# GabrieleCocco/CLFaceDetection

Hardware: NVIDIA B200
Metric: frames_per_sec_1080p (higher is better)
Workload: dtype f64

## Files before the change

clfacedetection_b200/csrc/haar_pack.cpp:

```cpp
#include <algorithm>
#include <cfloat>
#include <cmath>
#include <cstdarg>
#include <cstdio>
#include <cstdlib>
#include <cstring>

#include "clfd_pack.h"

namespace clfd {

static thread_local char g_error[1024] = "";

void set_error(const char *fmt, ...) {
    va_list ap;
    va_start(ap, fmt);
    vsnprintf(g_error, sizeof g_error, fmt, ap);
    va_end(ap);
}
const char *get_error() { return g_error; }

#define FMT_FAIL(...) do { set_error(__VA_ARGS__); return CLFD_ERR_FORMAT; } while (0)

int build_hidden(HostCascade &c) {
// ... 165 lines not shown
    L.eq_off[2] = (ey + eh) * pitch + ex; L.eq_off[3] = (ey + eh) * pitch + ex + ew;
    for (int n = 0; n < c.n_nodes(); n++) {
        const HostNode &nd = c.nodes[n];
        ScNode &d = out[n];
        memset(&d, 0, sizeof d);
        const int nr = c.hid_nrects[n];
        double sum0 = 0, area0 = 0;
        const double correction_ratio = weight_scale * (!nd.tilted ? 1 : 0.5);
        for (int k = 0; k < nr; k++) {
            const int tx = cv_round_d(nd.rect[k][0] * scale), tw = cv_round_d(nd.rect[k][2] * scale);
            const int ty = cv_round_d(nd.rect[k][1] * scale), th = cv_round_d(nd.rect[k][3] * scale);
            int dy[4], dx[4];
            if (!nd.tilted) {
                dy[0] = ty;      dx[0] = tx;
                dy[1] = ty;      dx[1] = tx + tw;
                dy[2] = ty + th; dx[2] = tx;
                dy[3] = ty + th; dx[3] = tx + tw;
            } else {
                dy[2] = ty + tw;      dx[2] = tx + tw;
                dy[3] = ty + tw + th; dx[3] = tx + tw - th;
                dy[0] = ty;           dx[0] = tx;
                dy[1] = ty + th;      dx[1] = tx - th;
            }
            for (int q = 0; q < 4; q++) d.off[k * 4 + q] = dy[q] * pitch + dx[q];
            d.w[k] = (float)(nd.weight[k] * correction_ratio);
            if (k == 0) area0 = tw * th;
            else sum0 += d.w[k] * tw * th;
        }
        d.w[0] = (float)(-sum0 / area0);
        d.thr = nd.threshold;
        d.left = nd.left; d.right = nd.right;
        d.flags = (nd.tilted ? 1 : 0) | (nr << 8);
    }
}

static void pack_dense_one(const HostCascade &c, int ystep, DenseParams &P, std::vector<TailStump> &tail,
                           std::vector<DenseStage> &stage_tab, int &dense_stumps, int patch_stride = 0,
                           bool allow_tiles = true) {
    const int S = c.n_stages(), T = c.n_trees();
    memset(&P, 0, sizeof P);
    P.total_stages = S;
    P.win_w = c.win_w; P.win_h = c.win_h;
    P.tile_stride = dense_tile_stride(c.win_w, ystep);
    P.tile_half = dense_tile_half(c.win_w, ystep);
    if (patch_stride > 0) { P.tile_stride = patch_stride; P.tile_half = 0; }
    P.is_tree = c.is_tree ? 1 : 0;
    P.ystep = ystep;
    P.filter_eps = 9.5367431640625e-07f;
    if (const char *e = getenv("CLFD_FORCE_EXACT")) P.force_exact = atoi(e) != 0;
    P.inv_area = 1. / ((c.win_w - 2) * (c.win_h - 2));
    P.eq_x = 1; P.eq_y = 1; P.eq_w = c.win_w - 2; P.eq_h = c.win_h - 2;
    P.tilted_tile = c.has_tilted && !getenv("CLFD_NO_TILTED_TILE") ? 1 : 0;
    P.tile_h = kTileH;
    if (P.tilted_tile && ystep == 2 && !c.is_tree && !getenv("CLFD_NO_SMALL_TILES")) P.tile_h = kTileHSmall;
    if (ystep == 2 && !P.tilted_tile && !c.is_tree && c.is_stump_based) {
        const char *e = getenv("CLFD_TILE_H2");
        if (!e || atoi(e) == 24) P.tile_h = 24;
    }
    const size_t tile_bytes = (size_t)dense_tile_rows(c.win_h, ystep, P.tile_h) * P.tile_stride * 4;
    const size_t tilt_base = (tile_bytes + 127) & ~(size_t)127;
    const bool dense_ok = allow_tiles && tile_bytes <= 65536 && (!P.tilted_tile || 2 * tilt_base <= 160 * 1024) && c.win_w <= 255 && c.win_h <= 255;
    int npt = 1;
    for (int t = 0; t < T; t++) npt = std::max(npt, c.tr_nnodes[t]);
    if (getenv("CLFD_NO_NODE_TILES") && npt > 1) npt = kMaxTreeNodes + 1;
    P.npt = npt <= kMaxTreeNodes ? npt : 1;
    auto stage_ok = [&](int i) {
// ... 75 lines not shown
                for (int k = 0; k < c.hid_nrects[n]; k++) {
                    int dx[4], dy[4];
                    corner_coords(nd, k, dx, dy);
                    for (int q = 0; q < 4; q++) ts.off[k * 4 + q] = tile_offset(dy[q], dx[q]) + (nd.tilted ? (uint32_t)tilt_base : 0u);
                    ts.w[k] = c.hid_weight[(size_t)n * 3 + k];
                }
                ts.thr = nd.threshold;
                ts.a0 = nd.left <= 0 ? c.alpha[a + (-nd.left)] : 0.f;
                ts.a1 = nd.right <= 0 ? c.alpha[a + (-nd.right)] : 0.f;
                ts.meta = (uint32_t)j | ((nd.left > 0 ? (uint32_t)nd.left : kNodeLeaf) << 8) |
                          ((nd.right > 0 ? (uint32_t)nd.right : kNodeLeaf) << 16);
                amax = fmax(amax, fmax(fabs((double)ts.a0), fabs((double)ts.a1)));
            }
            abs_sum += amax;
        }
        ds.first = 0; ds.count = (uint16_t)(c.st_ntrees[i] * P.npt);
        ds.thr = c.hid_thr[i];
        ds.flags = ((!c.is_tree && c.is_stump_based && c.two_rects[i]) ? 1u : 0u) | (any3 ? 2u : 0u) |
                   (c.order_free[i] ? 4u : 0u);
        const double er = (double)(c.st_ntrees[i] * P.npt) * ldexp(1.0, -23) * abs_sum;
        ds.sum_eps = std::isfinite(er) ? (float)(er * 1.0000002) + FLT_MIN : INFINITY;
        ds.sum_eps += 1.0001e-5f * std::fabs(ds.thr);
        if (walk_tree) {
            const uint32_t pass = c.st_child[i] >= 0 ? (uint32_t)pos[c.st_child[i]] : kRouteAccept;
            int p = i;
            while (p >= 0 && c.st_next[p] < 0) p = c.st_parent[p];
            const uint32_t fail = p >= 0 ? (uint32_t)pos[c.st_next[p]] : kRouteReject;
            ds.flags |= ((uint32_t)i << 8) | (pass << 16) | (fail << 24);
            stage_tab[e] = ds;
        }
        if (e < elig) P.stage[e] = ds;
    }
    const bool share_corners = !getenv("CLFD_NO_SHARED_CORNERS");
    int ns = 0, nstump = 0;
    while (ns < elig && nstump + c.st_ntrees[ns] * P.npt <= kMaxDenseStumps) {
        P.stage[ns].first = (uint16_t)nstump;
        std::vector<DenseStump> six, rest;
        for (int t = c.st_first_tree[ns] * P.npt; t < c.st_first_tree[ns + 1] * P.npt; t++) {
            DenseStump st = tail[t];
            bool shared = false;
            if (share_corners && P.npt == 1 && c.hid_nrects[c.tr_first_node[t]] == 2) {
                const uint32_t *A = st.off, *B = st.off + 4;
                static const int pairs[4][2] = {{0, 2}, {3, 1}, {0, 1}, {3, 2}};
                for (const auto &pr : pairs) {
                    const int pl = pr[0], mi = pr[1];
                    if (A[pl] != B[pl] || A[mi] != B[mi]) continue;
                    const int opl = pl == 0 ? 3 : 0, omi = mi == 1 ? 2 : 1;
                    const uint32_t o[6] = {A[pl], A[mi], A[opl], A[omi], B[opl], B[omi]};
                    for (int q = 0; q < 12; q++) st.off[q] = q < 6 ? o[q] : 0;
                    shared = true;
                    break;
                }
            }
            (shared ? six : rest).push_back(st);
        }
        P.stage[ns].n_shared = (uint32_t)six.size();
        for (const auto &st : six) P.stump[nstump++] = st;
        for (const auto &st : rest) P.stump[nstump++] = st;
        ns++;
    }
    P.n_stages = ns;
    {
        static_assert(sizeof(TailStump) == 80, "five 16-byte chunks per record");
        struct Chunk { uint32_t v[4]; };
        std::vector<TailStump> blocked;
        const Chunk *src = reinterpret_cast<const Chunk *>(tail.data());
        int at = 0;
        for (int e = 0; e < E; e++) {
            const int count = c.st_ntrees[order[e]] * P.npt;
            const size_t first = blocked.size();
            blocked.resize(first + (size_t)((count + 31) / 32) * 32);
            Chunk *blk = reinterpret_cast<Chunk *>(blocked.data() + first);
            for (int j = 0; j < count; j++)
                for (int q = 0; q < 5; q++) blk[(size_t)(j >> 5) * 160 + q * 32 + (j & 31)] = src[(size_t)(at + j) * 5 + q];
            if (e < elig) P.stage[e].tail_first = (uint32_t)first;
            if (walk_tree) stage_tab[e].tail_first = (uint32_t)first;
            at += count;
        }
        tail.swap(blocked);
    }
    P.pool_min = 0;
    if (const char *e = getenv("CLFD_POOL_MIN")) P.pool_min = std::max(0, atoi(e));
    P.track_abs = 0;
    for (float v : c.alpha)
        if (std::fabs(v) > 64.f) P.track_abs = 1;
    if (getenv("CLFD_NO_TRACK_ABS")) P.track_abs = 0;
// ... 100 lines not shown
```

clfacedetection_b200/csrc/kernels_clod.cu:

```cuda
#include <algorithm>
#include <cstdint>

#include "clfd_pack.h"
#include "kernels.h"

namespace clfd {

typedef unsigned long long ull;

__device__ __forceinline__ uint32_t smem_u32(const void *p) { return (uint32_t)__cvta_generic_to_shared(p); }

__device__ __forceinline__ void mbar_init(uint64_t *bar, uint32_t count) {
    asm volatile("mbarrier.init.shared::cta.b64 [%0], %1;" ::"r"(smem_u32(bar)), "r"(count));
    asm volatile("fence.mbarrier_init.release.cluster;" ::: "memory");
}
__device__ __forceinline__ void mbar_expect_tx(uint64_t *bar, uint32_t bytes) {
    asm volatile("mbarrier.arrive.expect_tx.shared::cta.b64 _, [%0], %1;" ::"r"(smem_u32(bar)), "r"(bytes) : "memory");
}
__device__ __forceinline__ void mbar_wait(uint64_t *bar, uint32_t parity) {
    asm volatile(
        "{\n"
        ".reg .pred P1;\n"
        "LAB_WAIT:\n"
        "mbarrier.try_wait.parity.shared::cta.b64 P1, [%0], %1;\n"
// ... 177 lines not shown
    const double sigma = dense_sigma(P, c, wid);
    const uint4 *rec = reinterpret_cast<const uint4 *>(P.tail + tail_first);
    double S = 0.0;
    uint32_t at = 0;
    for (int j = 0; j < count; j++) {
        const StumpRegs q = stump_from_global(rec, j, true);
        if (NODES) {
            if ((q.meta & 255u) == 0u) at = 0;
            if ((q.meta & 255u) != at) continue;
        }
        const int r0 = lds32(base + q.o[0]) - lds32(base + q.o[1]) - lds32(base + q.o[2]) + lds32(base + q.o[3]);
        const int r1 = lds32(base + q.o[4]) - lds32(base + q.o[5]) - lds32(base + q.o[6]) + lds32(base + q.o[7]);
        const double t = __dmul_rn((double)q.thr, sigma);
        double sum;
        if (dbl) {
            sum = __fma_rn((double)r1, (double)q.w1, __dmul_rn((double)r0, (double)q.w0));
        } else {
            sum = __dadd_rn((double)__fmul_rn(__int2float_rn(r0), q.w0), (double)__fmul_rn(__int2float_rn(r1), q.w1));
            if (q.o[11] != 0) {
                const int r2 = lds32(base + q.o[8]) - lds32(base + q.o[9]) - lds32(base + q.o[10]) + lds32(base + q.o[11]);
                sum = __dadd_rn(sum, (double)__fmul_rn(__int2float_rn(r2), q.w2));
            }
        }
        if (NODES) {
            at = ((sum >= t ? q.meta >> 16 : q.meta >> 8)) & 255u;
            if (at != kNodeLeaf) continue;
        }
        S = __dadd_rn(S, (double)(sum >= t ? q.a1 : q.a0));
    }
    const double thr = (double)sthr;
    return (S >= thr ? 1 : 0) | (fabs(__dsub_rn(S, thr)) <= __dmul_rn(1e-5, fabs(thr)) ? 2 : 0);
}

template <int KK, int K, bool FIXED, int ROWSTEP, bool SHARED, bool NODES, bool TRACK>
__device__ __forceinline__ void stump_filter_window(const StumpRegs &q, bool dbl, bool three, float eps, const uint32_t (&c)[12],
                                                    const uint32_t (&base)[K], const float (&sg)[K], float (&S)[K], bool (&near)[K],
                                                    uint32_t (&at)[K], float (&Sa)[K]) {
    const float eps4 = eps * 0.25f;
    constexpr int IMM = KK * ROWSTEP;
    const uint32_t b = base[FIXED ? 0 : KK];
    int r0, r1;
    if (SHARED) {
        int e, f, g;
        if (FIXED) {
            e = lds32i<IMM>(c[0]) - lds32i<IMM>(c[1]); f = lds32i<IMM>(c[2]) - lds32i<IMM>(c[3]); g = lds32i<IMM>(c[4]) - lds32i<IMM>(c[5]);
        } else {
            e = lds32(b + q.o[0]) - lds32(b + q.o[1]); f = lds32(b + q.o[2]) - lds32(b + q.o[3]); g = lds32(b + q.o[4]) - lds32(b + q.o[5]);
        }
        r0 = e + f; r1 = e + g;
    } else if (FIXED) {
        r0 = lds32i<IMM>(c[0]) - lds32i<IMM>(c[1]) - lds32i<IMM>(c[2]) + lds32i<IMM>(c[3]);
        r1 = lds32i<IMM>(c[4]) - lds32i<IMM>(c[5]) - lds32i<IMM>(c[6]) + lds32i<IMM>(c[7]);
    } else {
        r0 = lds32(b + q.o[0]) - lds32(b + q.o[1]) - lds32(b + q.o[2]) + lds32(b + q.o[3]);
        r1 = lds32(b + q.o[4]) - lds32(b + q.o[5]) - lds32(b + q.o[6]) + lds32(b + q.o[7]);
    }
    const float p0 = __fmul_rn(__int2float_rn(r0), q.w0);
    float s32 = __fmaf_rn(__int2float_rn(r1), q.w1, p0);
    float m = __fmaf_rn(fabsf(p0), eps4, __fmul_rn(fabsf(q.thr), __fmul_rn(sg[KK], eps)));
    if (!SHARED && three) {
        int r2;
        if (FIXED) r2 = lds32i<IMM>(c[8]) - lds32i<IMM>(c[9]) - lds32i<IMM>(c[10]) + lds32i<IMM>(c[11]);
        else r2 = lds32(b + q.o[8]) - lds32(b + q.o[9]) - lds32(b + q.o[10]) + lds32(b + q.o[11]);
        m = __fmaf_rn(fabsf(s32), eps4, m);
        s32 = __fmaf_rn(__int2float_rn(r2), q.w2, s32);
    }
    const float d = __fmaf_rn(-q.thr, sg[KK], s32);
    if (NODES) {
        const bool on = at[KK] == (q.meta & 255u);
        near[KK] = near[KK] || (on && fabsf(d) <= m);
        S[KK] = __fadd_rn(S[KK], on ? (d >= 0.f ? q.a1 : q.a0) : 0.f);
        at[KK] = on ? ((d >= 0.f ? q.meta >> 16 : q.meta >> 8) & 255u) : at[KK];
    } else {
        near[KK] = near[KK] || (fabsf(d) <= m);
        const float sel = d >= 0.f ? q.a1 : q.a0;
        S[KK] = __fadd_rn(S[KK], sel);
        if (TRACK) Sa[KK] = __fadd_rn(Sa[KK], fabsf(sel));
    }
}

template <int K, bool FIXED, int ROWSTEP, bool SHARED, bool NODES, bool TRACK>
__device__ __forceinline__ void stump_filter(const StumpRegs &q, bool dbl, bool any3, float eps, const uint32_t (&base)[K],
                                             const float (&sg)[K], float (&S)[K], bool (&near)[K], uint32_t (&at)[K], float (&Sa)[K]) {
    static_assert(K >= 1 && K <= 4, "1..4 windows per thread");
    const bool three = !SHARED && any3 && q.o[11] != 0u;
    uint32_t c[12];
    if (FIXED) {
#pragma unroll
        for (int i = 0; i < (SHARED ? 6 : 12); i++) c[i] = base[0] + q.o[i];
    }
    if (NODES && (q.meta & 255u) == 0u) {
#pragma unroll
        for (int k = 0; k < K; k++) at[k] = 0u;
    }
    stump_filter_window<0, K, FIXED, ROWSTEP, SHARED, NODES, TRACK>(q, dbl, three, eps, c, base, sg, S, near, at, Sa);
    if (K > 1) stump_filter_window<(K > 1 ? 1 : 0), K, FIXED, ROWSTEP, SHARED, NODES, TRACK>(q, dbl, three, eps, c, base, sg, S, near, at, Sa);
    if (K > 2) stump_filter_window<(K > 2 ? 2 : 0), K, FIXED, ROWSTEP, SHARED, NODES, TRACK>(q, dbl, three, eps, c, base, sg, S, near, at, Sa);
    if (K > 3) stump_filter_window<(K > 3 ? 3 : 0), K, FIXED, ROWSTEP, SHARED, NODES, TRACK>(q, dbl, three, eps, c, base, sg, S, near, at, Sa);
}

template <int K, bool FIXED, int ROWSTEP, bool NODES, bool TRACK>
__device__ __forceinline__ void stage_filter(const DenseParams &P, const DenseStage &st, bool resident, int grp, int G,
                                             const uint32_t (&base)[K], const float (&sg)[K], float (&S)[K], bool (&near)[K],
                                             float (&Sa)[K]) {
    uint32_t at[K];
#pragma unroll
    for (int k = 0; k < K; k++) at[k] = 0u;
    const int count = st.count;
    const uint32_t flags = st.flags;
    const bool dbl = flags & 1u, any3 = flags & 2u;
    const float eps = P.filter_eps;
    if (resident && G == 1) {
        const int first = st.first, n6 = (int)st.n_shared;
#pragma unroll 1
        for (int j = 0; j < n6; j++) stump_filter<K, FIXED, ROWSTEP, true, false, TRACK>(stump_from_param(P.stump[first + j]), dbl, false, eps, base, sg, S, near, at, Sa);
#pragma unroll 1
        for (int j = n6; j < count; j++) stump_filter<K, FIXED, ROWSTEP, false, NODES, TRACK>(stump_from_param(P.stump[first + j]), dbl, any3, eps, base, sg, S, near, at, Sa);
    } else {
        const uint4 *__restrict__ rec = reinterpret_cast<const uint4 *>(P.tail + st.tail_first);
        if (NODES) {
            const int npt = P.npt;
#pragma unroll 1
            for (int j = grp * npt; j < count; j += G * npt)
#pragma unroll 1
                for (int i = 0; i < npt; i++)
                    stump_filter<K, FIXED, ROWSTEP, false, true, TRACK>(stump_from_global(rec, j + i, any3), dbl, any3, eps, base, sg, S, near, at, Sa);
        } else {
#pragma unroll 1
            for (int j = grp; j < count; j += G) stump_filter<K, FIXED, ROWSTEP, false, false, TRACK>(stump_from_global(rec, j, any3), dbl, any3, eps, base, sg, S, near, at, Sa);
        }
    }
// ... 80 lines not shown
            if (tid == 0) mbar_init(bar, 1);
            __syncthreads();
            const uint32_t hb = (uint32_t)half * 4u;
            if (tid == 0) mbar_expect_tx(bar, (uint32_t)rows * 2u * hb);
            const int32_t *__restrict__ gdi = a.sum + frame_off + (size_t)py0 * L.sum_pitch + (px0 >> 1);
            for (int r = tid; r < rows * 2; r += kDenseThreads) {
                const int odd = r >= rows, rr = odd ? r - rows : r;
                tma_bulk_g2s(tile + (size_t)rr * S * 4 + (odd ? hb : 0u), gdi + (size_t)rr * L.sum_pitch + (odd ? (L.sum_pitch >> 1) : 0), hb, bar);
            }
        }
        const int c4 = cols >> 2, total = rows * c4;
        for (int i = (di ? total : 0) + tid; i < total * n_tiles_smem; i += kDenseThreads) {
            const int t2 = i >= total, ii = t2 ? i - total : i;
            const int r = ii / c4, cq = ii - r * c4;
            const int4 v = __ldg(reinterpret_cast<const int4 *>((t2 ? gtil : gsum) + (size_t)r * L.sum_pitch) + cq);
            int *row = reinterpret_cast<int *>(tile + (t2 ? tile2_off : 0)) + r * S;
            *reinterpret_cast<int2 *>(row + 2 * cq) = make_int2(v.x, v.z);
            *reinterpret_cast<int2 *>(row + half + 2 * cq) = make_int2(v.y, v.w);
        }
        __syncthreads();
        if (di) mbar_wait(bar, 0);
    }

    DenseCtx c;
    c.tile = smem_u32(tile); c.gsq = a.sq; c.sq_at = frame_off + (size_t)py0 * L.sum_pitch + px0; c.sq32 = a.sq32 != 0;
    c.codes = a.codes ? a.codes + (size_t)frame * a.windows_per_frame + CL.win_base : nullptr;
    c.sq_pitch = L.sum_pitch;
    c.row_mul = ystep * S * 4;
    c.ystep = ystep; c.S = S; c.half = P.tile_half;
    c.tx = tx; c.wy_tile = ty * TILE_H; c.nx = CL.nx;
    c.code_mul = P.is_tree ? 2 : 1;
    const float inf = __int_as_float(0x7f800000);

    constexpr int kRowsPerSlot = kDenseThreads / kTileW;
    const int wx = tid & (kTileW - 1), wy0 = tid / kTileW;
    uint32_t alive = 0;
#pragma unroll
    for (int k = 0; k < kDenseSlots; k++) {
        const int wy = wy0 + k * kRowsPerSlot;
        const int wid = wy * kTileW + wx;
        if (wx < n_wx && wy < n_wy) {
            bool eq_flat, live = true;
            sgf[wid] = (float)dense_sigma_flat(P, c, wid, eq_flat);
            if (!COUNT && eq_flat && P.flat_code) {
                const int code = flat_window_code(P, c, wid);
                if (code != kNotFlat) {
                    live = false;
                    if (P.is_tree ? (code & 1) : (code == P.total_stages)) emit_rect(a, CL, frame, px0 + wx * ystep, py0 + wy * ystep);
                }
            }
            if (live) alive |= 1u << k;
        } else {
            sgf[wid] = 1.0f;
        }
    }
    int s = 0;
    for (; s < P.n_fixed; s++) {
        const float sthr = P.stage[s].thr, seps = P.force_exact ? inf : P.stage[s].sum_eps;
#pragma unroll 1
        for (int k0 = 0; k0 < kDenseSlots; k0 += kDenseChunk) {
            const uint32_t m4 = (alive >> k0) & ((1u << kDenseChunk) - 1u);
            if (!__any_sync(0xffffffffu, m4 != 0)) continue;
            uint32_t base[kDenseChunk];
            float sg[kDenseChunk];
            float Ssum[kDenseChunk];
            bool near[kDenseChunk];
#pragma unroll
            for (int k = 0; k < kDenseChunk; k++) {
                const int wy = wy0 + (k0 + k) * kRowsPerSlot;
                base[k] = c.tile + (uint32_t)(wy * c.row_mul + wx * 4);
                sg[k] = sgf[wy * kTileW + wx];
                Ssum[k] = 0.f;
                near[k] = false;
            }
            float Sabs[kDenseChunk];
#pragma unroll
            for (int k = 0; k < kDenseChunk; k++) Sabs[k] = 0.f;
            if (ROWSTEP_T) stage_filter<kDenseChunk, true, ROWSTEP_T, NODES, TRACK>(P, P.stage[s], true, 0, 1, base, sg, Ssum, near, Sabs);
            else stage_filter<kDenseChunk, false, 0, NODES, TRACK>(P, P.stage[s], true, 0, 1, base, sg, Ssum, near, Sabs);
#pragma unroll
            for (int k = 0; k < kDenseChunk; k++) {
                if (!((m4 >> k) & 1u)) continue;
                const int wid = (wy0 + (k0 + k) * kRowsPerSlot) * kTileW + wx;
                if (!stage_verdict<NODES, COUNT, TRACK>(P, c, P.stage[s], sthr, seps, wid, Ssum[k], near[k], Sabs[k])) {
                    alive &= ~(1u << (k0 + k));
                    if (c.codes) dense_write_code(c, wid, s * c.code_mul);
                }
            }
        }
    }

    constexpr int kClassCap = kTileWindows / 32;
    constexpr int kSeg = kTileWindows / kDenseWarps;
    int n_alive;
    uint16_t *cur;
    if (kPooledStages && P.pool_min > 0) {
        uint16_t *cl_in = list, *cl_out = reinterpret_cast<uint16_t *>(smem_raw + plan.pool);
        int *cnt_in = ctl + kCtlCount, *cnt_out = ctl + kCtlCountB, *cnt_zero = ctl + kCtlCountC;
        {
            const int na = __popc(alive);
            if (na) {
                const int cq = (wx + 8 * wy0) & 31;
                int at = atomicAdd(cnt_in + cq, na);
    #pragma unroll
                for (int k = 0; k < kDenseSlots; k++)
                    if ((alive >> k) & 1u) cl_in[cq * kClassCap + at++] = (uint16_t)((wy0 + k * kRowsPerSlot) * kTileW + wx);
            }
        }
        __syncthreads();
            for (;; s++) {
            const int h = cnt_in[lane];
            int incl = h, hmax = h;
    #pragma unroll
            for (int d = 1; d < 32; d <<= 1) {
                const int v = __shfl_up_sync(0xffffffffu, incl, d);
                if (lane >= d) incl += v;
                hmax = max(hmax, __shfl_xor_sync(0xffffffffu, hmax, d));
            }
            const int excl = incl - h, tot = __shfl_sync(0xffffffffu, incl, 31);
            if (tot == 0) return;
            n_alive = tot;
            if (!(P.pool_min > 0 && tot > P.pool_min && s < P.tail_stages)) {
                for (int r = warp; r < h; r += kDenseWarps) {
                    const int i = excl + r;
                    const int w = i % kDenseWarps, p = i / kDenseWarps;
                    const int nw = (tot - w + kDenseWarps - 1) / kDenseWarps, Rw = (nw + 31) >> 5;
                    const int col = p / Rw, row = p - col * Rw;
                    cl_out[w * kSeg + row * 32 + col] = cl_in[lane * kClassCap + r];
                }
                __syncthreads();
                break;
            }
            int R = (tot + 31) >> 5;
            {
                int best = 0x7fffffff;
                for (int r = R; r <= hmax; r++) {
                    int e = max(h - r, 0);
    #pragma unroll
                    for (int d = 16; d > 0; d >>= 1) e += __shfl_xor_sync(0xffffffffu, e, d);
// ... 25 lines not shown
                }
                if (valid && !pass && c.codes) dense_write_code(c, wid, s * c.code_mul);
            };
            for (int r = r_begin; r < r_end; r += 2) {
                bool v0, v1 = false;
                const int wid0 = fetch(r, v0);
                if (r + 1 < r_end) {
                    const int wid1 = fetch(r + 1, v1);
                    const uint32_t base[2] = {dense_base(c, wid0), dense_base(c, wid1)};
                    const float sg[2] = {sgf[wid0], sgf[wid1]};
                    float Ssum[2] = {0.f, 0.f};
                    bool near[2] = {false, false};
                    float Sabs[2] = {0.f, 0.f};
                    stage_filter<2, false, 0, NODES, TRACK>(P, P.stage[s], s < P.n_stages, 0, 1, base, sg, Ssum, near, Sabs);
                    keep_pool(v0, wid0, Ssum[0], near[0], Sabs[0]);
                    keep_pool(v1, wid1, Ssum[1], near[1], Sabs[1]);
                } else {
                    const uint32_t base[1] = {dense_base(c, wid0)};
                    const float sg[1] = {sgf[wid0]};
                    float Ssum[1] = {0.f};
                    bool near[1] = {false};
                    float Sabs[1] = {0.f};
                    stage_filter<1, false, 0, NODES, TRACK>(P, P.stage[s], s < P.n_stages, 0, 1, base, sg, Ssum, near, Sabs);
                    keep_pool(v0, wid0, Ssum[0], near[0], Sabs[0]);
                }
            }
            __syncthreads();
            uint16_t *tl = cl_in; cl_in = cl_out; cl_out = tl;
            int *tc = cnt_in; cnt_in = cnt_out; cnt_out = cnt_zero; cnt_zero = tc;
        }

        cur = cl_out + warp * kSeg;
    } else {
        const int na = __popc(alive), cq = (wx + 8 * wy0) & 31;
        int at = na ? atomicAdd(ctl + kCtlCount + cq, na) : 0;
        __syncthreads();
        const int h = ctl[kCtlCount + lane];
        int incl = h;
#pragma unroll
        for (int d = 1; d < 32; d <<= 1) {
            const int v = __shfl_up_sync(0xffffffffu, incl, d);
            if (lane >= d) incl += v;
        }
        n_alive = __shfl_sync(0xffffffffu, incl, 31);
        if (n_alive == 0) return;
        at += __shfl_sync(0xffffffffu, incl - h, cq);
#pragma unroll
        for (int k = 0; k < kDenseSlots; k++) {
            if ((alive >> k) & 1u) {
                const int i = at++;
                const int w = i % kDenseWarps, p = i / kDenseWarps;
                const int nw = (n_alive - w + kDenseWarps - 1) / kDenseWarps, Rw = (nw + 31) >> 5;
                const int col = p / Rw, row = p - col * Rw;
                list[w * kSeg + row * 32 + col] = (uint16_t)((wy0 + k * kRowsPerSlot) * kTileW + wx);
            }
        }
        __syncthreads();
        cur = list + warp * kSeg;
    }

#ifdef CLFD_TILE_TIMING
    if (lane == 0) atomicAdd(&s_dense_t_p1, (unsigned int)(clock64() - t_start));
#endif
    int n = (n_alive - warp + kDenseWarps - 1) / kDenseWarps;
    bool dealt = true;
    for (; s < P.cut_stages && n > 0; s++) {
        const float sthr = P.stage[s].thr, seps = P.force_exact ? inf : P.stage[s].sum_eps;
        int n_next = 0;
        auto keep = [&](bool valid, int wid, float Ssum, bool near, float Sabs) {
            const bool pass = valid && stage_verdict<NODES, COUNT, TRACK>(P, c, P.stage[s], sthr, seps, wid, Ssum, near, Sabs);
            const unsigned m = __ballot_sync(0xffffffffu, pass);
            if (pass) cur[n_next + __popc(m & ((1u << lane) - 1u))] = (uint16_t)wid;
            n_next += __popc(m);
            if (valid && !pass && c.codes) dense_write_code(c, wid, s * c.code_mul);
        };
        if (n > P.g1_min) {
            const int R = (n + 31) >> 5;
            for (int r = 0; r < R; r += 2) {
                const int c0 = dealt ? (n - r + R - 1) / R : min(32, n - 32 * r);
                if (r + 1 < R) {
                    const int c1 = dealt ? (n - r - 1 + R - 1) / R : min(32, n - 32 * (r + 1));
                    const bool v0 = lane < c0, v1 = lane < c1;
                    const int wid0 = cur[32 * r + (v0 ? lane : 0)], wid1 = cur[32 * r + 32 + (v1 ? lane : 0)];
                    __syncwarp();
                    const uint32_t base[2] = {dense_base(c, wid0), dense_base(c, wid1)};
                    const float sg[2] = {sgf[wid0], sgf[wid1]};
                    float Ssum[2] = {0.f, 0.f};
// ... 135 lines not shown
            }
            __syncwarp();
        }
        return;
    }
    if (n == 0) return;
    ull qb = 0;
    if (s < P.total_stages) {
        if (lane == 0) qb = atomicAdd(a.qcount, (ull)n);
        qb = __shfl_sync(0xffffffffu, qb, 0);
    }
    const int Rn = (n + 31) >> 5;
    for (int idx = lane; idx < Rn * 32; idx += 32) {
        const int row = idx >> 5, col = idx & 31;
        if (col >= (dealt ? (n - row + Rn - 1) / Rn : min(32, n - 32 * row))) continue;
        const int i = dealt ? col * Rn + row : idx;
        const int w = cur[idx];
        const int x = px0 + (w & (kTileW - 1)) * ystep, y = py0 + (w / kTileW) * ystep;
        if (s >= P.total_stages) {
            emit_rect(a, CL, frame, x, y);
            if (c.codes) dense_write_code(c, w, P.total_stages);
        } else if (qb + i < a.queue_cap) {
            QueueItem it;
            it.key = ((uint32_t)frame << 16) | ((uint32_t)cl << 8) | (uint32_t)s;
            it.xy = ((uint32_t)y << 16) | (uint32_t)x;
            a.queue[qb + i] = it;
        } else {
            atomicAdd(a.counters + 3, 1ull);
        }
    }
}

template <int ROWSTEP_T, bool TREE, bool NODES, int TILE_H, bool COUNT, bool TRACK = false>
__global__ void __launch_bounds__(kDenseThreads)
k_cascade_tiles(const __grid_constant__ DenseParams P, const __grid_constant__ CascadeArgs a, const int tile0) {
    extern __shared__ __align__(128) unsigned char smem_raw[];
#ifdef CLFD_TILE_TIMING
    const long long t_cta = clock64();
#endif
    cascade_tiles_body<ROWSTEP_T, TREE, NODES, TILE_H, COUNT, TRACK>(P, a, tile0, smem_raw);
#ifdef CLFD_TILE_TIMING
    __syncwarp();
    if ((threadIdx.x & 31) == 0) {
        const unsigned int dt = (unsigned int)(clock64() - t_cta);
        atomicAdd(&s_dense_t_busy, dt);
        __threadfence_block();
        if (atomicAdd(&s_dense_done, 1u) == kDenseWarps - 1) {
            atomicAdd(a.counters + 4, (ull)s_dense_t_busy);
            atomicAdd(a.counters + 5, (ull)dt * kDenseWarps);
            atomicAdd(a.counters + 6, (ull)s_dense_t_p1);
        }
    }
    return;
#endif
    if (!COUNT) return;
    __syncwarp();
    if ((threadIdx.x & 31) == 0) {
        __threadfence_block();
        if (atomicAdd(&s_dense_done, 1u) == kDenseWarps - 1) {
            const unsigned int ne = s_dense_exact, nn = s_dense_near;
            if (ne) atomicAdd(a.counters + 4, (ull)ne);
            if (nn) atomicAdd(a.counters + 5, (ull)nn);
        }
    }
}

constexpr int kPatchWarps = 8;
// ... 111 lines not shown
            if (alive) emit_rect(a, CL, frame, x, y);
            if (c.codes) dense_write_code(c, 0, alive ? P.total_stages : s);
        }
        __syncwarp();
        q = qn;
    }
    if (!COUNT) return;
    __syncwarp();
    if (lane == 0) {
        __threadfence_block();
        if (atomicAdd(&s_dense_done, 1u) == kPatchWarps - 1) {
            const unsigned int ne = s_dense_exact, nn = s_dense_near;
            if (ne) atomicAdd(a.counters + 4, (ull)ne);
            if (nn) atomicAdd(a.counters + 5, (ull)nn);
        }
    }
}
static cudaError_t launch_patch_tt(const DenseParams &P, const CascadeArgs &a, int n_sms, cudaStream_t stream) {
    const size_t smem = (size_t)kPatchWarps * 2 * patch_buf_words(P) * 4;
    static SmemLimitCache limit;
    if (cudaError_t e = limit.ensure(k_cascade_patch<kTilesCount>, smem)) return e;
    const int per_sm = (int)std::max<size_t>(1, std::min<size_t>(4, (200 * 1024) / std::max<size_t>(smem, 1)));
    k_cascade_patch<kTilesCount><<<n_sms * per_sm, 32 * kPatchWarps, smem, stream>>>(P, a);
    return cudaGetLastError();
}

constexpr int dense_stride_ce(int win_w, int ystep) {
    int cols = ((kTileW - 1) * ystep + win_w + 1 + 3) & ~3;
    int s = ystep == 1 ? cols : 2 * ((cols / 2 + 3) & ~3);
    s = (s + 3) & ~3;
    while ((ystep * s) % 32 != 8) s += 4;
    return s;
}
constexpr int dense_rowstep_ce(int win_w, int ystep) { return (kDenseThreads / kTileW) * ystep * dense_stride_ce(win_w, ystep) * 4; }

template <int ROWSTEP_T, bool TREE, bool NODES, int TILE_H = kTileH>
static cudaError_t launch_tiles_tt(const DenseParams &P, const CascadeArgs &a, int tile0, int n_tiles, size_t smem, cudaStream_t stream) {
    if constexpr (ROWSTEP_T == 0 && !TREE && !NODES) {
        if (P.track_abs) {
            static SmemLimitCache limit_track;
            if (cudaError_t e = limit_track.ensure(k_cascade_tiles<0, false, false, TILE_H, kTilesCount, true>, smem)) return e;
            k_cascade_tiles<0, false, false, TILE_H, kTilesCount, true><<<dim3(n_tiles, a.n_frames), kDenseThreads, smem, stream>>>(P, a, tile0);
            return cudaGetLastError();
        }
    }
    static SmemLimitCache limit;
    if (cudaError_t e = limit.ensure(k_cascade_tiles<ROWSTEP_T, TREE, NODES, TILE_H, kTilesCount>, smem)) return e;
    k_cascade_tiles<ROWSTEP_T, TREE, NODES, TILE_H, kTilesCount><<<dim3(n_tiles, a.n_frames), kDenseThreads, smem, stream>>>(P, a, tile0);
    return cudaGetLastError();
}
template <int ROWSTEP_T>
static cudaError_t launch_tiles_t(const DenseParams &P, const CascadeArgs &a, int tile0, int n_tiles, size_t smem, cudaStream_t stream) {
    constexpr int R = ROWSTEP_T;
    if (P.exec_stages > P.tail_stages) return launch_tiles_tt<R, true, false>(P, a, tile0, n_tiles, smem, stream);
    if (P.tile_h == kTileHSmall) {
        if (P.npt > 1) return launch_tiles_tt<R, false, true, kTileHSmall>(P, a, tile0, n_tiles, smem, stream);
        return launch_tiles_tt<R, false, false, kTileHSmall>(P, a, tile0, n_tiles, smem, stream);
    }
    if (P.tile_h == 24) {
        if (P.exec_stages > P.tail_stages || P.npt > 1) return cudaErrorInvalidValue;
        return launch_tiles_tt<ROWSTEP_T, false, false, 24>(P, a, tile0, n_tiles, smem, stream);
    }
    if (P.tile_h != kTileH) return cudaErrorInvalidValue;
    if (P.npt > 1) return launch_tiles_tt<R, false, true>(P, a, tile0, n_tiles, smem, stream);
    return launch_tiles_tt<ROWSTEP_T, false, false>(P, a, tile0, n_tiles, smem, stream);
}

#ifdef CLFD_TILES_COUNT_TU
cudaError_t launch_cascade_patch_count(const DenseParams &P, const CascadeArgs &a, int n_sms, cudaStream_t stream) {
    return launch_patch_tt(P, a, n_sms, stream);
}
#else
cudaError_t launch_cascade_patch_count(const DenseParams &P, const CascadeArgs &a, int n_sms, cudaStream_t stream);
cudaError_t launch_cascade_patch(const DenseParams &P, const CascadeArgs &a, int n_sms, cudaStream_t stream) {
    if (a.n_frames == 0) return cudaSuccess;
    return a.count_exact ? launch_cascade_patch_count(P, a, n_sms, stream) : launch_patch_tt(P, a, n_sms, stream);
}
#endif
#ifdef CLFD_TILES_COUNT_TU
cudaError_t launch_cascade_tiles_count(const DenseParams &P, const CascadeArgs &a, int tile0, int n_tiles, cudaStream_t stream) {
#else
cudaError_t launch_cascade_tiles_count(const DenseParams &P, const CascadeArgs &a, int tile0, int n_tiles, cudaStream_t stream);
cudaError_t launch_cascade_tiles(const DenseParams &P, const CascadeArgs &a, int tile0, int n_tiles, cudaStream_t stream) {
    if (a.count_exact) return launch_cascade_tiles_count(P, a, tile0, n_tiles, stream);
#endif
    if (n_tiles <= 0 || a.n_frames == 0) return cudaSuccess;
    const size_t smem = dense_smem_plan(P).total;
    const int rowstep = (kDenseThreads / kTileW) * P.ystep * P.tile_stride * 4;
    constexpr int r20_1 = dense_rowstep_ce(20, 1), r20_2 = dense_rowstep_ce(20, 2);
    constexpr int r24_1 = dense_rowstep_ce(24, 1), r24_2 = dense_rowstep_ce(24, 2);
    static_assert(r20_1 == r24_1 && r20_2 == r24_2 && r20_2 != r20_1, "row steps must be distinct switch labels");
    if (P.track_abs && P.exec_stages <= P.tail_stages && P.npt == 1) return launch_tiles_t<0>(P, a, tile0, n_tiles, smem, stream);
    switch (rowstep) {
        case r20_1: return launch_tiles_t<r20_1>(P, a, tile0, n_tiles, smem, stream);
        case r20_2: return launch_tiles_t<r20_2>(P, a, tile0, n_tiles, smem, stream);
        default:    return launch_tiles_t<0>(P, a, tile0, n_tiles, smem, stream);
    }
}

#ifndef CLFD_TILES_COUNT_TU
__global__ void __launch_bounds__(256) k_enqueue_all(const CascadeArgs a) {
    const long long w = (long long)blockIdx.x * 256 + threadIdx.x;
    const int frame = blockIdx.y;
    if (w == 0 && frame == 0) a.counters[1] = (ull)a.windows_per_frame * a.n_frames;
    if (w >= a.windows_per_frame) return;
    int lo = 0, hi = a.n_cas_levels - 1;
    while (lo < hi) {
        const int mid = (lo + hi + 1) >> 1;
        if (__ldg(&a.cas_levels[mid].win_base) <= w) lo = mid; else hi = mid - 1;
    }
    const int nx = __ldg(&a.cas_levels[lo].nx), ystep = __ldg(&a.cas_levels[lo].ystep);
    const int local = (int)(w - __ldg(&a.cas_levels[lo].win_base));
    const int iy = local / nx, ix = local - iy * nx;
    QueueItem it;
    it.key = ((uint32_t)frame << 16) | ((uint32_t)lo << 8);
    it.xy = ((uint32_t)(iy * ystep) << 16) | (uint32_t)(ix * ystep);
    a.queue[(size_t)frame * a.windows_per_frame + w] = it;
}

cudaError_t launch_enqueue_all(const CascadeArgs &a, cudaStream_t stream) {
    if (a.windows_per_frame == 0 || a.n_frames == 0) return cudaSuccess;
// ... 279 lines not shown
```

Measured before the change: 2852.

## Assign consecutive window rows per thread and reuse rectangle pair sums across rows

Each thread now handles vertically adjacent windows instead of rows strided by the thread-row count, so per-slot row offset becomes a single ystep row. The host packer computes a per-stump descriptor recording when one rectangle corner-pair difference equals another pair shifted down by 1-3 rows. In the fixed-offset kernel path, already loaded pair differences from earlier slots are reused instead of reloaded from shared memory. This cuts shared-memory loads but adds registers (h[6][K]); launch bounds now request min-blocks occupancy. The compaction class assignment is also reworked for the new mapping.

After: 2558, median of 6. -10.3%, worse.

```diff
diff --git a/clfacedetection_b200/csrc/haar_pack.cpp b/clfacedetection_b200/csrc/haar_pack.cpp
--- a/clfacedetection_b200/csrc/haar_pack.cpp
+++ b/clfacedetection_b200/csrc/haar_pack.cpp
@@ -221,6 +221,20 @@
         d.left = nd.left; d.right = nd.right;
         d.flags = (nd.tilted ? 1 : 0) | (nr << 8);
     }
+}
+
+static uint32_t reuse_descriptor(const uint32_t off[12], bool six, int64_t row_bytes) {
+    auto shift = [&](int p, int s) -> uint32_t {
+        const int64_t d0 = (int64_t)off[2 * s] - off[2 * p], d1 = (int64_t)off[2 * s + 1] - off[2 * p + 1];
+        if (d0 != d1 || d0 <= 0 || d0 % row_bytes != 0 || d0 / row_bytes > 3) return 0u;
+        return (uint32_t)(d0 / row_bytes);
+    };
+    if (six) {
+        uint32_t mef = shift(0, 1), meg = shift(0, 2);
+        if (mef && meg) (mef <= meg ? meg : mef) = 0u;
+        return mef | (meg << 2) | (shift(1, 0) << 4) | (shift(2, 0) << 6);
+    }
+    return shift(0, 1) | (shift(2, 3) << 2) | (off[11] != 0u ? shift(4, 5) << 4 : 0u);
 }
 
 static void pack_dense_one(const HostCascade &c, int ystep, DenseParams &P, std::vector<TailStump> &tail,
@@ -362,6 +376,7 @@
         if (e < elig) P.stage[e] = ds;
     }
     const bool share_corners = !getenv("CLFD_NO_SHARED_CORNERS");
+    const int64_t row_bytes = (int64_t)ystep * P.tile_stride * 4;
     int ns = 0, nstump = 0;
     while (ns < elig && nstump + c.st_ntrees[ns] * P.npt <= kMaxDenseStumps) {
         P.stage[ns].first = (uint16_t)nstump;
@@ -376,12 +391,13 @@
                     const int pl = pr[0], mi = pr[1];
                     if (A[pl] != B[pl] || A[mi] != B[mi]) continue;
                     const int opl = pl == 0 ? 3 : 0, omi = mi == 1 ? 2 : 1;
-                    const uint32_t o[6] = {A[pl], A[mi], A[opl], A[omi], B[opl], B[omi]};
+                    const uint32_t o[6] = {A[pl], A[mi], A[omi], A[opl], B[omi], B[opl]};
                     for (int q = 0; q < 12; q++) st.off[q] = q < 6 ? o[q] : 0;
                     shared = true;
                     break;
                 }
             }
+            if (P.npt == 1) st.meta = reuse_descriptor(st.off, shared, row_bytes);
             (shared ? six : rest).push_back(st);
         }
         P.stage[ns].n_shared = (uint32_t)six.size();
diff --git a/clfacedetection_b200/csrc/kernels_clod.cu b/clfacedetection_b200/csrc/kernels_clod.cu
--- a/clfacedetection_b200/csrc/kernels_clod.cu
+++ b/clfacedetection_b200/csrc/kernels_clod.cu
@@ -233,22 +233,60 @@
     return (S >= thr ? 1 : 0) | (fabs(__dsub_rn(S, thr)) <= __dmul_rn(1e-5, fabs(thr)) ? 2 : 0);
 }
 
+constexpr uint32_t kMaxPairShift = 2u;
+template <int KK>
+__device__ __forceinline__ bool pair_reusable(uint32_t m) { return KK > 0 && m != 0u && m <= (uint32_t)KK && m <= kMaxPairShift; }
+template <int KK, int K>
+__device__ __forceinline__ int pair_from(const int (&h)[K], uint32_t m) {
+    int v = h[KK >= 1 ? KK - 1 : 0];
+    if (KK >= 2 && m == 2u) v = h[KK >= 2 ? KK - 2 : 0];
+    if (KK >= 3 && kMaxPairShift >= 3 && m == 3u) v = h[KK >= 3 ? KK - 3 : 0];
+    return v;
+}
+template <int KK, int K, int ROWSTEP, int PP>
+__device__ __forceinline__ int pair_load(const uint32_t (&c)[12], int (&h)[6][K]) {
+    const int v = lds32i<KK * ROWSTEP>(c[2 * PP]) - lds32i<KK * ROWSTEP>(c[2 * PP + 1]);
+    h[PP][KK] = v;
+    return v;
+}
+template <int KK, int K, int ROWSTEP, int PP, int SRC>
+__device__ __forceinline__ int pair_reuse(const uint32_t (&c)[12], int (&h)[6][K], uint32_t m) {
+    if (pair_reusable<KK>(m)) {
+        const int v = pair_from<KK, K>(h[SRC], m);
+        h[PP][KK] = v;
+        return v;
+    }
+    return pair_load<KK, K, ROWSTEP, PP>(c, h);
+}
+
 template <int KK, int K, bool FIXED, int ROWSTEP, bool SHARED, bool NODES, bool TRACK>
 __device__ __forceinline__ void stump_filter_window(const StumpRegs &q, bool dbl, bool three, float eps, const uint32_t (&c)[12],
                                                     const uint32_t (&base)[K], const float (&sg)[K], float (&S)[K], bool (&near)[K],
-                                                    uint32_t (&at)[K], float (&Sa)[K]) {
+                                                    uint32_t (&at)[K], float (&Sa)[K], int (&h)[6][K]) {
     const float eps4 = eps * 0.25f;
     constexpr int IMM = KK * ROWSTEP;
+    constexpr bool REUSE = FIXED && !NODES;
     const uint32_t b = base[FIXED ? 0 : KK];
     int r0, r1;
     if (SHARED) {
         int e, f, g;
-        if (FIXED) {
+        if (REUSE) {
+            const uint32_t d = q.meta, mef = d & 3u, meg = (d >> 2) & 3u;
+            if (pair_reusable<KK>(mef)) { e = pair_from<KK, K>(h[1], mef); h[0][KK] = e; }
+            else if (pair_reusable<KK>(meg)) { e = pair_from<KK, K>(h[2], meg); h[0][KK] = e; }
+            else e = pair_load<KK, K, ROWSTEP, 0>(c, h);
+            f = pair_reuse<KK, K, ROWSTEP, 1, 0>(c, h, (d >> 4) & 3u);
+            g = pair_reuse<KK, K, ROWSTEP, 2, 0>(c, h, (d >> 6) & 3u);
+        } else if (FIXED) {
             e = lds32i<IMM>(c[0]) - lds32i<IMM>(c[1]); f = lds32i<IMM>(c[2]) - lds32i<IMM>(c[3]); g = lds32i<IMM>(c[4]) - lds32i<IMM>(c[5]);
         } else {
             e = lds32(b + q.o[0]) - lds32(b + q.o[1]); f = lds32(b + q.o[2]) - lds32(b + q.o[3]); g = lds32(b + q.o[4]) - lds32(b + q.o[5]);
         }
-        r0 = e + f; r1 = e + g;
+        r0 = e - f; r1 = e - g;
+    } else if (REUSE) {
+        const uint32_t d = q.meta;
+        r0 = pair_reuse<KK, K, ROWSTEP, 0, 1>(c, h, d & 3u) - pair_load<KK, K, ROWSTEP, 1>(c, h);
+        r1 = pair_reuse<KK, K, ROWSTEP, 2, 3>(c, h, (d >> 2) & 3u) - pair_load<KK, K, ROWSTEP, 3>(c, h);
     } else if (FIXED) {
         r0 = lds32i<IMM>(c[0]) - lds32i<IMM>(c[1]) - lds32i<IMM>(c[2]) + lds32i<IMM>(c[3]);
         r1 = lds32i<IMM>(c[4]) - lds32i<IMM>(c[5]) - lds32i<IMM>(c[6]) + lds32i<IMM>(c[7]);
@@ -261,7 +299,8 @@
     float m = __fmaf_rn(fabsf(p0), eps4, __fmul_rn(fabsf(q.thr), __fmul_rn(sg[KK], eps)));
     if (!SHARED && three) {
         int r2;
-        if (FIXED) r2 = lds32i<IMM>(c[8]) - lds32i<IMM>(c[9]) - lds32i<IMM>(c[10]) + lds32i<IMM>(c[11]);
+        if (REUSE) r2 = pair_reuse<KK, K, ROWSTEP, 4, 5>(c, h, (q.meta >> 4) & 3u) - pair_load<KK, K, ROWSTEP, 5>(c, h);
+        else if (FIXED) r2 = lds32i<IMM>(c[8]) - lds32i<IMM>(c[9]) - lds32i<IMM>(c[10]) + lds32i<IMM>(c[11]);
         else r2 = lds32(b + q.o[8]) - lds32(b + q.o[9]) - lds32(b + q.o[10]) + lds32(b + q.o[11]);
         m = __fmaf_rn(fabsf(s32), eps4, m);
         s32 = __fmaf_rn(__int2float_rn(r2), q.w2, s32);
@@ -294,10 +333,11 @@
 #pragma unroll
         for (int k = 0; k < K; k++) at[k] = 0u;
     }
-    stump_filter_window<0, K, FIXED, ROWSTEP, SHARED, NODES, TRACK>(q, dbl, three, eps, c, base, sg, S, near, at, Sa);
-    if (K > 1) stump_filter_window<(K > 1 ? 1 : 0), K, FIXED, ROWSTEP, SHARED, NODES, TRACK>(q, dbl, three, eps, c, base, sg, S, near, at, Sa);
-    if (K > 2) stump_filter_window<(K > 2 ? 2 : 0), K, FIXED, ROWSTEP, SHARED, NODES, TRACK>(q, dbl, three, eps, c, base, sg, S, near, at, Sa);
-    if (K > 3) stump_filter_window<(K > 3 ? 3 : 0), K, FIXED, ROWSTEP, SHARED, NODES, TRACK>(q, dbl, three, eps, c, base, sg, S, near, at, Sa);
+    int h[6][K];
+    stump_filter_window<0, K, FIXED, ROWSTEP, SHARED, NODES, TRACK>(q, dbl, three, eps, c, base, sg, S, near, at, Sa, h);
+    if (K > 1) stump_filter_window<(K > 1 ? 1 : 0), K, FIXED, ROWSTEP, SHARED, NODES, TRACK>(q, dbl, three, eps, c, base, sg, S, near, at, Sa, h);
+    if (K > 2) stump_filter_window<(K > 2 ? 2 : 0), K, FIXED, ROWSTEP, SHARED, NODES, TRACK>(q, dbl, three, eps, c, base, sg, S, near, at, Sa, h);
+    if (K > 3) stump_filter_window<(K > 3 ? 3 : 0), K, FIXED, ROWSTEP, SHARED, NODES, TRACK>(q, dbl, three, eps, c, base, sg, S, near, at, Sa, h);
 }
 
 template <int K, bool FIXED, int ROWSTEP, bool NODES, bool TRACK>
@@ -444,12 +484,11 @@
     c.code_mul = P.is_tree ? 2 : 1;
     const float inf = __int_as_float(0x7f800000);
 
-    constexpr int kRowsPerSlot = kDenseThreads / kTileW;
-    const int wx = tid & (kTileW - 1), wy0 = tid / kTileW;
+    const int wx = tid & (kTileW - 1), wy1 = (tid / kTileW) * kDenseSlots;
     uint32_t alive = 0;
 #pragma unroll
     for (int k = 0; k < kDenseSlots; k++) {
-        const int wy = wy0 + k * kRowsPerSlot;
+        const int wy = wy1 + k;
         const int wid = wy * kTileW + wx;
         if (wx < n_wx && wy < n_wy) {
             bool eq_flat, live = true;
@@ -479,7 +518,7 @@
             bool near[kDenseChunk];
 #pragma unroll
             for (int k = 0; k < kDenseChunk; k++) {
-                const int wy = wy0 + (k0 + k) * kRowsPerSlot;
+                const int wy = wy1 + k0 + k;
                 base[k] = c.tile + (uint32_t)(wy * c.row_mul + wx * 4);
                 sg[k] = sgf[wy * kTileW + wx];
                 Ssum[k] = 0.f;
@@ -493,7 +532,7 @@
 #pragma unroll
             for (int k = 0; k < kDenseChunk; k++) {
                 if (!((m4 >> k) & 1u)) continue;
-                const int wid = (wy0 + (k0 + k) * kRowsPerSlot) * kTileW + wx;
+                const int wid = (wy1 + k0 + k) * kTileW + wx;
                 if (!stage_verdict<NODES, COUNT, TRACK>(P, c, P.stage[s], sthr, seps, wid, Ssum[k], near[k], Sabs[k])) {
                     alive &= ~(1u << (k0 + k));
                     if (c.codes) dense_write_code(c, wid, s * c.code_mul);
@@ -504,19 +543,23 @@
 
     constexpr int kClassCap = kTileWindows / 32;
     constexpr int kSeg = kTileWindows / kDenseWarps;
+    constexpr int kClassesPerThread = kDenseSlots < 4 ? kDenseSlots : 4;
+    constexpr uint32_t kClassSlots = 0x11u;
     int n_alive;
     uint16_t *cur;
     if (kPooledStages && P.pool_min > 0) {
         uint16_t *cl_in = list, *cl_out = reinterpret_cast<uint16_t *>(smem_raw + plan.pool);
         int *cnt_in = ctl + kCtlCount, *cnt_out = ctl + kCtlCountB, *cnt_zero = ctl + kCtlCountC;
         {
-            const int na = __popc(alive);
-            if (na) {
-                const int cq = (wx + 8 * wy0) & 31;
-                int at = atomicAdd(cnt_in + cq, na);
     #pragma unroll
-                for (int k = 0; k < kDenseSlots; k++)
-                    if ((alive >> k) & 1u) cl_in[cq * kClassCap + at++] = (uint16_t)((wy0 + k * kRowsPerSlot) * kTileW + wx);
+            for (int j = 0; j < kClassesPerThread; j++) {
+                const uint32_t mine = alive & (kClassSlots << j);
+                if (!mine) continue;
+                const int cq = (wx + 8 * (wy1 + j)) & 31;
+                int at = atomicAdd(cnt_in + cq, __popc(mine));
+    #pragma unroll
+                for (int k = j; k < kDenseSlots; k += 4)
+                    if ((mine >> k) & 1u) cl_in[cq * kClassCap + at++] = (uint16_t)((wy1 + k) * kTileW + wx);
             }
         }
         __syncthreads();
@@ -608,8 +651,12 @@
 
         cur = cl_out + warp * kSeg;
     } else {
-        const int na = __popc(alive), cq = (wx + 8 * wy0) & 31;
-        int at = na ? atomicAdd(ctl + kCtlCount + cq, na) : 0;
+        int at[kClassesPerThread];
+#pragma unroll
+        for (int j = 0; j < kClassesPerThread; j++) {
+            const int na = __popc(alive & (kClassSlots << j));
+            at[j] = na ? atomicAdd(ctl + kCtlCount + ((wx + 8 * (wy1 + j)) & 31), na) : 0;
+        }
         __syncthreads();
         const int h = ctl[kCtlCount + lane];
         int incl = h;
@@ -620,15 +667,17 @@
         }
         n_alive = __shfl_sync(0xffffffffu, incl, 31);
         if (n_alive == 0) return;
-        at += __shfl_sync(0xffffffffu, incl - h, cq);
+#pragma unroll
+        for (int j = 0; j < kClassesPerThread; j++)
+            at[j] += __shfl_sync(0xffffffffu, incl - h, (wx + 8 * (wy1 + j)) & 31);
 #pragma unroll
         for (int k = 0; k < kDenseSlots; k++) {
             if ((alive >> k) & 1u) {
-                const int i = at++;
+                const int i = at[k & 3]++;
                 const int w = i % kDenseWarps, p = i / kDenseWarps;
                 const int nw = (n_alive - w + kDenseWarps - 1) / kDenseWarps, Rw = (nw + 31) >> 5;
                 const int col = p / Rw, row = p - col * Rw;
-                list[w * kSeg + row * 32 + col] = (uint16_t)((wy0 + k * kRowsPerSlot) * kTileW + wx);
+                list[w * kSeg + row * 32 + col] = (uint16_t)((wy1 + k) * kTileW + wx);
             }
         }
         __syncthreads();
@@ -830,7 +879,7 @@
 }
 
 template <int ROWSTEP_T, bool TREE, bool NODES, int TILE_H, bool COUNT, bool TRACK = false>
-__global__ void __launch_bounds__(kDenseThreads)
+__global__ void __launch_bounds__(kDenseThreads, TREE || (TRACK && TILE_H != 24) ? 3 : NODES ? 0 : 4)
 k_cascade_tiles(const __grid_constant__ DenseParams P, const __grid_constant__ CascadeArgs a, const int tile0) {
     extern __shared__ __align__(128) unsigned char smem_raw[];
 #ifdef CLFD_TILE_TIMING
@@ -1008,7 +1057,7 @@
     while ((ystep * s) % 32 != 8) s += 4;
     return s;
 }
-constexpr int dense_rowstep_ce(int win_w, int ystep) { return (kDenseThreads / kTileW) * ystep * dense_stride_ce(win_w, ystep) * 4; }
+constexpr int dense_rowstep_ce(int win_w, int ystep) { return ystep * dense_stride_ce(win_w, ystep) * 4; }
 
 template <int ROWSTEP_T, bool TREE, bool NODES, int TILE_H = kTileH>
 static cudaError_t launch_tiles_tt(const DenseParams &P, const CascadeArgs &a, int tile0, int n_tiles, size_t smem, cudaStream_t stream) {
@@ -1062,7 +1111,7 @@
 #endif
     if (n_tiles <= 0 || a.n_frames == 0) return cudaSuccess;
     const size_t smem = dense_smem_plan(P).total;
-    const int rowstep = (kDenseThreads / kTileW) * P.ystep * P.tile_stride * 4;
+    const int rowstep = P.ystep * P.tile_stride * 4;
     constexpr int r20_1 = dense_rowstep_ce(20, 1), r20_2 = dense_rowstep_ce(20, 2);
     constexpr int r24_1 = dense_rowstep_ce(24, 1), r24_2 = dense_rowstep_ce(24, 2);
     static_assert(r20_1 == r24_1 && r20_2 == r24_2 && r20_2 != r20_1, "row steps must be distinct switch labels");
```
